# BjarkeHautop/bayesSSM

Hardware: AMD Instinct MI355X
Metric: particle-steps/sec (N x T), bootstrap filter (higher is better)
Workload: dtype f64; 1 GPU; BASELINE C2: linear-Gaussian SSM, bootstrap filter, T=1000, N=1048576, SISR + systematic resampling, return_particles=FALSE, device generator; per_gpu=one independent filter replica per GPU (no data-path collective), backend=single process

## Files before the change

bayesssm_amd/_lib.py:

```python
import contextlib
import ctypes as C
import os
import threading

_HERE = os.path.dirname(os.path.abspath(__file__))
LIB_PATH = os.environ.get("BAYESSSM_AMD_LIB") or os.path.join(_HERE, "libbayesssm_amd.so")

OK, ERR_NEGATIVE, ERR_ZERO_SUM, ERR_LENGTH, ERR_ARG, ERR_HIP, ERR_CAPACITY = range(7)
MODEL = {"lg": 0, "ar1sin": 1, "sir": 2, "lgmv": 3, "rnet": 6}
MV_OBS_MODEL = {"gaussian": 3, "poisson": 4, "logvar": 5}
RN_OBS_MODEL = {"poisson": 6, "negbin": 7}
ALGORITHM = {"BPF": 0, "APF": 1, "RMPF": 2}
RESAMPLE_ALGORITHM = {"SIS": 0, "SISR": 1, "SISAR": 2}
RESAMPLE_FN = {"stratified": 0, "systematic": 1, "multinomial": 2, "multinomial_r": 3}
TRANSFORM = {"identity": 0, "log": 1, "logit": 2}
PRIOR = {"normal": 0, "exponential": 1, "uniform": 2, "flat": 3, "halfnormal": 4}


class BssmError(RuntimeError):
    def __init__(self, status, message):
        super().__init__(message)
        self.status = status


# ... 65 lines not shown
    lib.bssm_last_error.restype = C.c_char_p
    lib.bssm_status_string.restype = C.c_char_p
    lib.bssm_status_string.argtypes = [C.c_int]
    lib.bssm_ctx_stream.restype = C.c_void_p
    lib.bssm_ctx_stream.argtypes = [C.c_void_p]
    lib.bssm_ctx_create.argtypes = [C.c_int, C.c_longlong, C.c_int, C.POINTER(C.c_void_p)]
    lib.bssm_ctx_destroy.argtypes = [C.c_void_p]
    lib.bssm_ctx_destroy.restype = None
    lib.bssm_ctx_synchronize.argtypes = [C.c_void_p]
    lib.bssm_ctx_set_profile.argtypes = [C.c_void_p, C.c_int]
    lib.bssm_ctx_set_option.argtypes = [C.c_void_p, C.c_int, C.c_int]
    lib.bssm_ctx_get_stamps.argtypes = [C.c_void_p, C.c_void_p]
    if hasattr(lib, "bssm_ctx_fused_stats"):
        lib.bssm_ctx_fused_stats.argtypes = [C.c_void_p, C.c_void_p]
        lib.bssm_ctx_fused_stamps.argtypes = [C.c_void_p, C.c_void_p]
    if hasattr(lib, "bssm_ctx_multi_stats"):
        lib.bssm_ctx_multi_stats.argtypes = [C.c_void_p, C.c_void_p]
    lib.bssm_ctx_get_profile.argtypes = [C.c_void_p, C.c_int, C.c_void_p, C.c_void_p, C.c_void_p]
    lib.bssm_resample_ex.argtypes = [C.c_void_p, C.c_int, C.c_int, C.c_void_p, C.c_int, C.c_void_p,
                                     C.c_void_p, C.c_void_p, C.c_void_p]
    lib.bssm_resample_systematic.argtypes = [C.c_void_p, C.c_int, C.c_void_p, C.c_int, C.c_double, C.c_void_p]
    lib.bssm_resample_stratified.argtypes = [C.c_void_p, C.c_int, C.c_void_p, C.c_int, C.c_void_p, C.c_void_p]
    lib.bssm_resample_multinomial.argtypes = [C.c_void_p, C.c_int, C.c_void_p, C.c_int, C.c_void_p, C.c_void_p]
    lib.bssm_resample_multinomial_r.argtypes = [C.c_void_p, C.c_int, C.c_void_p, C.c_int, C.c_void_p, C.c_void_p]
    lib.bssm_resample_device.argtypes = [C.c_void_p, C.c_int, C.c_int, C.c_void_p, C.c_int, C.c_double,
                                         C.c_void_p, C.c_void_p, C.c_void_p]
    lib.bssm_resample_device_status.argtypes = [C.c_void_p]
    lib.bssm_pf_run.argtypes = [C.c_void_p, C.POINTER(PfConfig), C.POINTER(PfResult)]
    lib.bssm_pf_noise_shape.argtypes = [C.c_int, C.c_int, C.c_void_p, C.POINTER(C.c_int), C.POINTER(C.c_int)]
    lib.bssm_dump_normals.argtypes = [C.c_void_p, C.c_ulonglong, C.c_ulonglong, C.c_int, C.c_int, C.c_longlong, C.c_void_p]
# ... 23 lines not shown
        lib.bssm_pf_run_batch_tv.argtypes = [C.c_void_p, C.POINTER(PfConfig), C.c_int, C.c_void_p, C.c_void_p, C.c_void_p,
                                             C.POINTER(MvTvBatch), C.POINTER(PfBatchResult)]
    _lib = lib
    return lib


EXPORTED_SYMBOLS = [
    "bssm_ctx_create", "bssm_ctx_destroy", "bssm_last_error", "bssm_status_string", "bssm_device_count",
    "bssm_ctx_synchronize", "bssm_ctx_stream", "bssm_resample_systematic", "bssm_resample_stratified",
    "bssm_resample_multinomial", "bssm_resample_device", "bssm_resample_device_status", "bssm_resample_ex",
    "bssm_pf_run", "bssm_pf_noise_shape", "bssm_dump_normals", "bssm_dump_uniforms", "bssm_dump_move_draws",
    "bssm_ctx_set_profile", "bssm_ctx_get_profile", "bssm_ctx_set_option", "bssm_ctx_get_stamps", "bssm_pmmh_chain",
    "bssm_resample_multinomial_r",
    "bssm_pf_run_batch", "bssm_pf_run_batch_tv", "bssm_pf_batch_max_particles", "bssm_pf_batch_max_particles_mv", "bssm_pf_batch_max_particles_rn", "bssm_rn_nb_tables", "bssm_pmmh_chains_batch", "bssm_pmmh_chain_draws",
    "bssm_pf_run_sharded", "bssm_pf_weigh_resample", "bssm_ctx_fused_stats", "bssm_ctx_fused_stamps", "bssm_dump_normals_mv", "bssm_dump_move_draws_mv", "bssm_pf_run_multi", "bssm_pmmh_chains_multi",
    "bssm_ctx_multi_stats", "bssm_dump_rpois", "bssm_dump_rbinom", "bssm_dump_rgamma",
]


def check(status):
    if status != OK:
        lib = load()
        msg = lib.bssm_last_error().decode() or lib.bssm_status_string(status).decode()
        raise BssmError(status, msg)


class Context:

    def __init__(self, device=0, max_particles=1 << 20, max_dim=1):
        lib = load()
        if lib.bssm_device_count() <= 0:
# ... 8 lines not shown
        if os.environ.get("BAYESSSM_AMD_FUSED") is not None:
            check(lib.bssm_ctx_set_option(h, 9, int(os.environ["BAYESSSM_AMD_FUSED"])))
        if os.environ.get("BAYESSSM_AMD_FUSED_PREFETCH") is not None:
            check(lib.bssm_ctx_set_option(h, 10, int(os.environ["BAYESSSM_AMD_FUSED_PREFETCH"])))

    @property
    def handle(self):
        return self._h

    def synchronize(self):
        check(load().bssm_ctx_synchronize(self._h))

    OPTIONS = {"record_window": 1, "batch_literal_max": 2, "stage_expansion": 3, "inkernel_resolve": 4, "debug_stop": 5, "fuse_step": 6, "renormalize": 7, "recompute_lw": 8, "fused": 9, "fused_prefetch": 10,
               "force_fallback": 11, "fused_tag": 12, "mv_y_missing": 13, "rn_leaps": 14, "fused_early_max": 0}

    QUALIFIERS = {"rn_method": OPTIONS["rn_leaps"] + 1, "rn_noise": OPTIONS["rn_leaps"] + 2}

    def set_option(self, name, value):
        check(load().bssm_ctx_set_option(self._h, self.OPTIONS[name] if name in self.OPTIONS else self.QUALIFIERS[name], int(value)))
        self._set_options[name] = int(value)

    @contextlib.contextmanager
    def mv_y_missing(self, skip):
        if not skip:
            yield
            return
        before = self._set_options.get("mv_y_missing", 0)
        self.set_option("mv_y_missing", 1)
        try:
            yield
        finally:
# ... 21 lines not shown
                    self.set_option("rn_method", method)
                if noise != before_noise:
                    self.set_option("rn_noise", noise)
                yield
            finally:
                if self._set_options.get("rn_noise", 0) != before_noise:
                    self.set_option("rn_noise", before_noise)
                if self._set_options.get("rn_method", 0) != before:
                    self.set_option("rn_method", before)

    def fused_stats(self):
        out = (C.c_longlong * 4)()
        check(load().bssm_ctx_fused_stats(self._h, out))
        return {"runs": out[0], "launches": out[1], "stand_downs": out[2], "timeouts": out[3]}

    def multi_stats(self):
        out = (C.c_longlong * 2)()
        check(load().bssm_ctx_multi_stats(self._h, out))
        return {"lockstep": out[0], "sequential": out[1]}

    def set_profile(self, enable):
        check(load().bssm_ctx_set_profile(self._h, 1 if enable else 0))

    def get_profile(self):
        n = 64
        names = (C.c_char_p * n)()
        ms = (C.c_double * n)()
        cnt = (C.c_longlong * n)()
        k = load().bssm_ctx_get_profile(self._h, n, names, ms, cnt)
        return {names[i].decode(): {"ms": ms[i], "launches": cnt[i]} for i in range(k)}
# ... 43 lines not shown
```

bayesssm_amd/csrc/bssm_api.hip:

```cpp
#include <hip/hip_runtime.h>
#include <hip/hip_ext.h>
#include <math.h>
#include <stdio.h>
#include <string.h>
#include <string>
#include <vector>
#include <map>
#include <algorithm>
#include "kernels.hip.h"
#include "fused.hip.h"
#include "mv.hip.h"
#include "rnet.hip.h"
#include "multi.hip.h"
#include <atomic>
#include "../../include/bayesssm_amd.h"

using namespace bssm;

static thread_local std::string g_err;

#define HIPCHK(expr)                                                                      \
    do {                                                                                  \
        hipError_t e__ = (expr);                                                          \
        if (e__ != hipSuccess) {                                                          \
// ... 17 lines not shown
    BlockRec *brec = nullptr, *brec_p = nullptr;
    SideList *side = nullptr, *side_p = nullptr;
    uint64_t* cin = nullptr;
    DevState* st = nullptr;
    unsigned long long* gmax_cur = nullptr;
    int sh_boff = 0, sh_nloc = 0;
    int opt_window = 0;
    int opt_batch_lit_max = 384;
    int opt_stage = 1;
    int opt_inkernel_resolve = 1;
    int opt_renormalize = 1;
    int opt_recompute_lw = 1;
    int opt_fuse_step = 0;
    int opt_debug_stop = 0;
    int opt_fused_prefetch = 0;
    int opt_fused_early_max = 1;
    int opt_force_fallback = 0;
    int opt_mv_y_missing = 0;
    int opt_rn_leaps = 0;
    int opt_rn_noise = 0;
    int opt_rn_method = 0;
    int opt_fused = 1;
    FusedWs* fz = nullptr; uint32_t fz_tag = 0; bool fz_ok = false;
    long long fz_launches = 0, fz_runs = 0, fz_bails = 0, fz_timeouts = 0;
    long long multi_lockstep = 0, multi_sequential = 0;
    std::map<std::string, std::pair<void*, size_t>> pool;
    hipEvent_t ev0 = nullptr, ev1 = nullptr;
    void* h_stage = nullptr; size_t h_stage_bytes = 0;
    bool profile = false;
    std::map<std::string, ProfEntry> prof;
// ... 169 lines not shown
    switch (option) {
        case BSSM_OPT_RN_NOISE: c->opt_rn_noise = value; break;
        case BSSM_OPT_RN_LEAPS: c->opt_rn_leaps = value; break;
        case BSSM_OPT_RN_METHOD: c->opt_rn_method = value; break;
        case BSSM_OPT_RECORD_WINDOW: c->opt_window = value; break;
        case BSSM_OPT_BATCH_LITERAL_MAX: c->opt_batch_lit_max = value; break;
        case BSSM_OPT_STAGE_EXPANSION: c->opt_stage = value; break;
        case BSSM_OPT_INKERNEL_RESOLVE: c->opt_inkernel_resolve = value; break;
        case BSSM_OPT_DEBUG_STOP: c->opt_debug_stop = value; break;
        case BSSM_OPT_FUSE_STEP: c->opt_fuse_step = value; break;
        case BSSM_OPT_RECOMPUTE_LW: c->opt_recompute_lw = value ? 1 : 0; break;
        case BSSM_OPT_RENORMALIZE: c->opt_renormalize = value ? 1 : 0; break;
        case BSSM_OPT_FUSED: c->opt_fused = value < 0 ? 0 : (value > 2 ? 2 : value); break;
        case BSSM_OPT_FUSED_PREFETCH: c->opt_fused_prefetch = value ? 1 : 0; break;
        case BSSM_OPT_FUSED_EARLY_MAX: c->opt_fused_early_max = value ? 1 : 0; break;
        case BSSM_OPT_MV_Y_MISSING: c->opt_mv_y_missing = value ? 1 : 0; break;
        case BSSM_OPT_FORCE_FALLBACK: {
            if (value < 0 || value > (FF_SERIAL_WALK | FF_GENERAL_LINK | FF_SUM_PASS_ONLY)) ARGFAIL("bssm_ctx_set_option: force_fallback takes the bits 1 | 2 | 4");
            const int32_t v = value;
            HIPCHK(hipSetDevice(c->device));
            HIPCHK(hipMemcpyAsync(&c->st->force_fallback, &v, sizeof(v), hipMemcpyHostToDevice, c->stream));
            HIPCHK(hipStreamSynchronize(c->stream));
            c->opt_force_fallback = value;
            break;
        }
        case BSSM_OPT_FUSED_TAG: {
            if (!c->fz) ARGFAIL("bssm_ctx_set_option: this context has no fused workspace");
            HIPCHK(hipSetDevice(c->device));
            HIPCHK(hipMemsetAsync(c->fz, 0, sizeof(FusedWs), c->stream));
            HIPCHK(hipStreamSynchronize(c->stream));
// ... 542 lines not shown
            if (cfg->return_particles)
                LAUNCH(c, "k_record_history", k_record_history, (unsigned)((N + 255) / 256), 256, 0, X0, c->w, N, dim,
                       (double*)d_ph + (size_t)i * N * dim, (double*)d_wh + (size_t)i * N, c->st);
        };
        if (fused) {
            for (int step = 1; step < gap; step++) { launch_step_model(c, cfg->model, true, 0, false, X0, N, B, par, yi, noise(ktrans)); ktrans++; }
            FusedArgs g;
            g.xin = X0; g.N = N; g.nblk = B; g.par = par; g.y = yi; g.trans = (gap >= 1) ? 1 : 0; g.ns = noise(gap >= 1 ? ktrans : 0);
            if (gap >= 1) ktrans++;
            g.obs_i = i; g.resample_algorithm = resample_algorithm; g.threshold = threshold;
            g.ess_out = (double*)d_ess; g.llh_out = (double*)d_llh; g.resampled_out = (int*)d_resampled;
            g.w_out = cfg->return_particles ? c->w : nullptr;
            g.lim = c->opt_window > 0 ? c->opt_window : rec_window(N);
            g.force_fallback = c->opt_force_fallback;
            g.early_max = c->opt_fused_early_max;
            ApplyArgs& a = g.a;
            a.w = c->w; a.nw = N; a.ain_p = c->ain_p; a.cin = c->cin; a.lim = g.lim; a.n = (int)N;
            a.u_base = (const double*)d_ur; a.u_stride = u_stride; a.key = key;
            a.anc_out = (int*)d_anc; a.anc_stride = N; a.cum_out = nullptr;
            a.xsrc = X0; a.xdst = X1; a.dim = 1; a.xstride = N; a.auxsrc = nullptr; a.auxdst = nullptr;
            a.se_part = se_row;
            a.nstage = (c->opt_stage && !d_anc) ? 1 : 0; a.lead = 0; a.last = B - 1;
            a.step_model = -1; a.step_par = par; a.step_y = 0; a.step_ns = g.ns; a.step_lw = nullptr;
            g.ws = c->fz; g.tag = ++c->fz_tag;
            if (g.tag == 0) {
                HIPCHK(hipMemsetAsync(c->fz, 0, sizeof(FusedWs), c->stream));
                g.tag = c->fz_tag = 1;
            }
            g.znext = nullptr; g.znext_call = 0;
            if (z_ready) { g.ns.arr = z_ready; z_ready = nullptr; }
// ... 611 lines not shown
    HIPCHK(hipMemcpy(out, c->fz->pubt, sizeof(c->fz->pubt), hipMemcpyDeviceToHost));
    return BSSM_OK;
}

extern "C" int bssm_ctx_fused_waket(bssm_ctx* c, long long* out )
{
    if (!c || !out || !c->fz) ARGFAIL("bssm_ctx_fused_waket: NULL argument");
    HIPCHK(hipMemcpy(out, c->fz->waket, sizeof(c->fz->waket), hipMemcpyDeviceToHost));
    return BSSM_OK;
}

extern "C" int bssm_ctx_fused_stats(bssm_ctx* c, long long* out )
{
    if (!c || !out) ARGFAIL("bssm_ctx_fused_stats: NULL argument");
    out[0] = c->fz_runs; out[1] = c->fz_launches; out[2] = c->fz_bails; out[3] = c->fz_timeouts;
    return BSSM_OK;
}

extern "C" int bssm_ctx_multi_stats(bssm_ctx* c, long long* out )
{
    if (!c || !out) ARGFAIL("bssm_ctx_multi_stats: NULL argument");
    out[0] = c->multi_lockstep; out[1] = c->multi_sequential;
    return BSSM_OK;
}

extern "C" int bssm_pf_run_multi(bssm_ctx* const* ctxs, int n_filters, const bssm_pf_config* cfg, const double* thetas,
                                 const unsigned long long* seeds, const unsigned long long* streams, bssm_pf_batch_result* res)
{
    if (!ctxs || !cfg || !res || !thetas || !seeds || !streams) ARGFAIL("bssm_pf_run_multi: NULL argument");
    const int F = n_filters;
// ... 1003 lines not shown
```

bayesssm_amd/csrc/fused.hip.h:

```cpp
#pragma once
#include "kernels.hip.h"

namespace bssm {

typedef unsigned long long fz_u64;
#define BSSM_RLX_AGENT __ATOMIC_RELAXED, __HIP_MEMORY_SCOPE_AGENT

constexpr int FZ_MAXB = 2 * NT;
constexpr int FZ_MINB = 256;
constexpr int FZ_KREC = 8;
constexpr int FZ_KSIDE = (int)(sizeof(SideEntry) / 4);
constexpr int FZ_NREP = 16;
constexpr int FZ_MAXSIDE = 16;
constexpr uint32_t FLAG_FUSED_BAIL = 8u, FLAG_FUSED_TIMEOUT = 16u;
constexpr uint32_t FZ_ST_DOIT = 1u, FZ_ST_DEAD = 2u, FZ_ST_STOP = 4u, FZ_ST_BAIL = 8u;
constexpr long long FZ_TIMEOUT_TICKS = 2000000ll;

struct FusedWs {
    fz_u64 e1[6][FZ_MAXB];
    fz_u64 c1[FZ_NREP][16];
    fz_u64 m1[FZ_NREP][16];
    fz_u64 s1[FZ_NREP][16];
    fz_u64 a1[2][FZ_MAXB];
    fz_u64 e2[FZ_KREC][FZ_MAXB];
    fz_u64 c2[FZ_NREP][16];
    fz_u64 e3[FZ_KREC][FZ_MAXB];
    fz_u64 c3[FZ_NREP][16];
    fz_u64 a3[2][FZ_MAXB];
    fz_u64 side_w[FZ_MAXB][FZ_MAXSIDE][FZ_KSIDE];
    fz_u64 side_p[FZ_MAXB][FZ_MAXSIDE][FZ_KSIDE];
    BlockRec brec_priv[2][MAXB];
    SideList side_priv[2][FZ_MAXB];
    long long stamps[2][24];
    long long startt[FZ_MAXB];
    long long endt[FZ_MAXB];
    long long waket[5][FZ_MAXB];
    long long pubt[4][FZ_MAXB];
};

#ifdef BSSM_DEV_STAMPS
#define FZ_STAMP(k) do { if (fz_stamper) g.ws->stamps[fz_row][k] = clock64(); } while (0)
#else
#define FZ_STAMP(k) do { } while (0)
#endif

__device__ __forceinline__ fz_u64 fz_gran(uint32_t tag, uint32_t v) { return ((fz_u64)tag << 32) | v; }
__device__ __forceinline__ void fz_put(fz_u64* g, uint32_t tag, uint32_t v) { __hip_atomic_store(g, fz_gran(tag, v), BSSM_RLX_AGENT); }
__device__ __forceinline__ void fz_put64(fz_u64* g, uint32_t tag, uint64_t v) { fz_put(g, tag, (uint32_t)v); fz_put(g + 1, tag, (uint32_t)(v >> 32)); }
__device__ __forceinline__ void fz_put64x(fz_u64* g, int stride, uint32_t tag, uint64_t v) { fz_put(g, tag, (uint32_t)v); fz_put(g + stride, tag, (uint32_t)(v >> 32)); }
__device__ __forceinline__ fz_u64 fz_get(const fz_u64* g) { return __hip_atomic_load(g, BSSM_RLX_AGENT); }

__device__ __forceinline__ void fz_encode(const BlockRec& br, uint32_t (&w)[FZ_KREC])
// ... 67 lines not shown
            for (int k = 0; k < EL; k++) c = c + terms[tt * EL + k];
        }
        atomicAdd((unsigned long long*)&st->stat_serial_walks, 1ull);
        atomicAdd((unsigned long long*)&st->stat_literal_terms, (unsigned long long)EB);
    }
    __syncthreads();
}
__device__ __forceinline__ LaneTerms fz_lane_terms(const double (&v)[EL])
{
    LaneTerms r;
#pragma unroll
    for (int k = 0; k < EL; k++) r.a[k] = v[k];
    return r;
}

struct FusedRecSink {
    fz_u64* rec_planes;
    fz_u64* side_base;
    int bidx; uint32_t tag;
    double* terms; DevState* st;
    __device__ __forceinline__ void rec(const BlockRec& br) const
    {
        uint32_t w[FZ_KREC];
        fz_encode(br, w);
#pragma unroll
        for (int k = 0; k < FZ_KREC; k++) fz_put(rec_planes + (size_t)k * FZ_MAXB + bidx, tag, w[k]);
    }
    __device__ __forceinline__ void side(int k, const SideEntry& e) const
    {
        if (k >= FZ_MAXSIDE) return;
        uint32_t w[FZ_KSIDE];
// ... 2 lines not shown
#pragma unroll
        for (int q = 0; q < FZ_KSIDE; q++) fz_put(dst + q, tag, w[q]);
    }
    __device__ __forceinline__ void literal(uint64_t* tin, uint64_t cin, const double (&v)[EL]) const { fz_block_literal(tin, cin, terms, fz_lane_terms(v), st); }
};

struct FusedArgs {
    const double* xin;
    long long N; int nblk;
    ModelPar par; double y; NoiseSrc ns; int trans;
    int obs_i, resample_algorithm; double threshold;
    double* ess_out; double* llh_out; int* resampled_out;
    double* w_out;
    int lim;
    int force_fallback;
    int early_max;
    ApplyArgs a;
    FusedWs* ws; uint32_t tag;
    double* znext; uint32_t znext_call;
};

struct FusedSmem {
    double red[16]; double redq[16];
    uint32_t slot[16];
    int bail;
    int book; double ess1;
};

template <int NG>
__device__ __forceinline__ bool fz_gather(const fz_u64* planes, int c0, int c1, uint32_t tag, const FzClock& clk, int* bail, uint32_t (&w0)[NG], uint32_t (&w1)[NG])
// ... 452 lines not shown
        double acc0 = 0.0;
#pragma unroll
        for (int r = 0; r < EL; r++) {
            const long long j = b0 + t + NT * r;
            if (j < N) { const double x0 = xa[t + NT * r]; g.a.xdst[j] = x0; acc0 += x0 * wa[t + NT * r]; }
        }
        acc0 = block_sum(acc0, sm.sh4);
        if (t == 0) g.a.se_part[bidx] = acc0;
        book_late();
        fz_draw_next(g, j0, N);
        return;
    }
    if (status & FZ_ST_STOP) { book_late(); return; }
    FZ_STAMP(6);
    FusedRecSink sink; sink.bidx = bidx; sink.tag = g.tag; sink.terms = lx; sink.st = st;
    {
        BlockScan bsw;
        block_scan<MODE_W>(sm, v, a_in, g.lim, bsw);
        __syncthreads();
        sink.rec_planes = &g.ws->e2[0][0]; sink.side_base = &g.ws->side_w[0][0][0];
        block_record_tail<MODE_W, 11>(sm, tin, bsw, v, a_in, g.lim, st, 0, false, sink);
    }
    FZ_STAMP(7); FZ_PUBT(1);
    book_late();
    if (!resolver) fz_draw_next(g, j0, N);
    ResolveSmem& rs = *reinterpret_cast<ResolveSmem*>(dyn);
    uint64_t* cin_lds = reinterpret_cast<uint64_t*>(reinterpret_cast<char*>(dyn) + ((sizeof(ResolveSmem) + 15) / 16) * 16);
    if (resolver) {
        __syncthreads();
        bool bail = false;
        const uint64_t fin = fz_resolve_duty<MODE_W, false>(sm, rs, fs, g, st, clk, nullptr, bail);
        uint32_t stw = 0;
        if (bail) { stw = FZ_ST_BAIL; if (t == 0) atomicOr(&st->flags, fs.bail == 1 ? FLAG_FUSED_TIMEOUT : FLAG_FUSED_BAIL); }
        else {
// ... 24 lines not shown
        if (fs.slot[2] & (FZ_ST_BAIL | FZ_ST_STOP)) return;
        total = b2d(mk64(fs.slot[0], fs.slot[1]));
    }
    FZ_STAMP(11); FZ_WAKE(1);
    const double a_in_p = a_in / total;
#pragma unroll
    for (int k = 0; k < EL; k++) v[k] = v[k] / total;
    BlockScan bs;
#ifdef BSSM_DEV_STAMPS
    const bool xstamper = (t == 0 && bidx == B / 4);
    const int xdbg = 99;
    if (xstamper) st->stamps[2][10] = clock64();
#else
    const bool xstamper = false; const int xdbg = 0;
#endif
    block_scan<MODE_P>(sm, v, a_in_p, g.lim, bs);
    __syncthreads();
#ifdef BSSM_DEV_STAMPS
    if (xstamper) st->stamps[2][11] = clock64();
#endif
    sink.rec_planes = &g.ws->e3[0][0]; sink.side_base = &g.ws->side_p[0][0][0];
    block_record_tail<MODE_P, 3>(sm, tin, bs, v, a_in_p, g.lim, st, xdbg, xstamper, sink);
#ifdef BSSM_DEV_STAMPS
    if (xstamper) { st->stamps[2][9] = clock64(); st->stamps[2][8] = bs.nb; }
#endif
    FZ_STAMP(12); FZ_PUBT(2);
    uint64_t cinb = 0;
    if (resolver) {
        __syncthreads();
        bool bail = false;
        (void)fz_resolve_duty<MODE_P, true>(sm, rs, fs, g, st, clk, cin_lds, bail);
        uint32_t stp = 0;
        if (bail) { stp = FZ_ST_BAIL; if (t == 0) atomicOr(&st->flags, fs.bail == 1 ? FLAG_FUSED_TIMEOUT : FLAG_FUSED_BAIL); }
        for (int b = t; b < B; b += NT) fz_put64x(&g.ws->a3[0][b], FZ_MAXB, g.tag, bail ? 0ull : cin_lds[b]);
// ... 56 lines not shown
```

bayesssm_amd/csrc/kernels.hip.h:

```cpp
#pragma once
#include <hip/hip_runtime.h>
#include <stdint.h>
#include <math.h>
#include "seqsum.h"
#include "rng.h"

namespace bssm {

#ifndef BSSM_NT
#define BSSM_NT 256
#endif
#ifndef BSSM_EL
#define BSSM_EL 8
#endif
constexpr int NT = BSSM_NT;
constexpr int EL = BSSM_EL;
constexpr int NWV = NT / 64;
static_assert(NT * EL == 2048 && (NT == 256 || NT == 512) , "a scan workgroup covers 2048 terms with 4 or 8 waves");
constexpr int EB = NT * EL;
constexpr int MAXB = 2048;

typedef double v2d_nt __attribute__((ext_vector_type(2)));
#ifndef BSSM_ST_W
#define BSSM_ST_W 0
// ... 579 lines not shown
    int j = 0;
#pragma unroll 1
    for (; j < nent; j++) {
        const bool bad = (sv + w.nref) >= w.range;
        const uint32_t lo = (uint32_t)sv;
        const uint64_t k01 = (lo & 1u) ? w.K1 : w.K0, k23 = (lo & 1u) ? w.K3 : w.K2;
        const uint64_t out = ((sv & ~3ull) >> (w.sh & 63)) + ((lo & 2u) ? k23 : k01);
        if (__builtin_amdgcn_readlane((int)bad, j)) break;
        if (lane == j) { my_s = sv; my_out = out; }
        sv = readlane_u64(out, j);
    }
    s = sv;
    return j;
}

__device__ __forceinline__ int64_t shfl_up_i64(int64_t v, int off)
{
    int lo = (int)(uint32_t)(uint64_t)v, hi = (int)(uint32_t)((uint64_t)v >> 32);
    lo = __shfl_up(lo, off, 64); hi = __shfl_up(hi, off, 64);
    return (int64_t)(((uint64_t)(uint32_t)hi << 32) | (uint32_t)lo);
}

struct SegSmem {
    Pure wagg[16]; int wflag[16]; int wnb[16]; Pure wcarry[17]; int wsegbase[17];
    Pure bnd_excl[MAXBND]; Rec bnd_rec[MAXBND]; int bnd_lane[MAXBND]; uint64_t bnd_ent[MAXBND];
    double bnd_terms[MAXBND][EL];
    uint64_t seg_start[MAXBND + 1];
    int red_min[NWV][2], red_max[NWV][2];
    uint64_t segbase[MAXBND + 1];
    int wlastb[16];
// ... 146 lines not shown
{
    double c = b2d(in);
    for (long long j = j0; j < j1; j++) c = c + term_at<MODE>(w, nw, total, j);
    return d2b(c);
}

struct BlockScan {
    Rec leaf;
    Pure pleaf;
    Pure exc;
    Pure last_seg;
    bool isb;
    int seg, nb;
};

template <int MODE>
__device__ __forceinline__ void block_scan(SegSmem& sm, const double (&v)[EL], double a_in, int lim, BlockScan& bs)
{
    double ts = 0.0;
#pragma unroll
    for (int k = 0; k < EL; k++) ts += v[k];
    const double h = a_in + block_excl_scan(ts, sm.sh4);
    bs.leaf = chunk_record_fixed<EL>(v, h, lim);
    bs.isb = bs.leaf.kind != REC_PURE;
    bs.pleaf.d0 = (int64_t)(bs.leaf.o[0] - bs.leaf.base);
    bs.pleaf.d1 = (int64_t)(bs.leaf.o[1] - (bs.leaf.base + 1));
    bool prev_b = false;
    bs.exc = seg_excl_scan<NT / 64>(sm, bs.pleaf, bs.isb, bs.seg, bs.nb, bs.last_seg, &prev_b);
    if (!bs.isb && prev_b && bs.seg <= MAXBND) sm.segbase[bs.seg] = bs.leaf.base;
    if (bs.isb && bs.seg < MAXBND) {
        Rec& d = sm.bnd_rec[bs.seg];
        d.base = bs.leaf.base; d.o[0] = bs.leaf.o[0]; d.o[1] = bs.leaf.o[1]; d.o[2] = bs.leaf.o[2]; d.o[3] = bs.leaf.o[3];
        d.kind = bs.leaf.kind; d.lo = bs.leaf.lo; d.hi = bs.leaf.hi; d.pad = 0;
        sm.bnd_excl[bs.seg].d0 = bs.exc.d0; sm.bnd_excl[bs.seg].d1 = bs.exc.d1; sm.bnd_lane[bs.seg] = threadIdx.x;
#pragma unroll
        for (int q = 0; q < EL; q++) sm.bnd_terms[bs.seg][q] = v[q];
    }
}

template <int MODE>
__device__ __forceinline__ bool block_resolve(SegSmem& sm, const BlockScan& bs, uint64_t cin, int lim,
                                              const double* __restrict__ w, long long nw, double total, long long b0,
                                              uint64_t& ent)
{
    const int t = threadIdx.x;
    if (t == 0) sm.fail = (bs.nb > MAXBND) ? 1 : 0;
    __syncthreads();
    if (t < 64 && bs.nb == 0) {
        if (t == 0) sm.seg_start[0] = cin;
    } else if (t < 64 && bs.nb <= MAXBND) {
        const int lane = t, nb = bs.nb;
        Rec rec = rec_identity(0);
        Pure ex; ex.d0 = 0; ex.d1 = 0;
        if (lane < nb) { rec = sm.bnd_rec[lane]; ex = sm.bnd_excl[lane]; }
        const StepFn fn = stepfn_build(ex, rec);
        uint64_t s = cin, my_s = 0, my_out = 0;
        const WalkFn wfn = walkfn_from(fn, lane < nb);
        const int j0 = walk_chain_regs(wfn, nb, s, my_s, my_out);
        for (int j = j0; j < nb; j++) {
            bool ok;
            uint64_t o = stepfn_apply(fn, s, ok);
            if (!__builtin_amdgcn_readlane((int)ok, j)) {
                double c = b2d(pure_step(ex, s));
#pragma unroll
                for (int q = 0; q < EL; q++) c = c + sm.bnd_terms[j][q];
                o = d2b(c);
            }
            if (lane == j) { my_s = s; my_out = o; }
            const int olo = __builtin_amdgcn_readlane((int)(uint32_t)o, j), ohi = __builtin_amdgcn_readlane((int)(uint32_t)(o >> 32), j);
            s = ((uint64_t)(uint32_t)ohi << 32) | (uint32_t)olo;
        }
        const uint64_t my_ent = pure_step(ex, my_s);
        if (lane == 0) sm.seg_start[0] = cin;
        if (lane < nb) { sm.bnd_ent[lane] = my_ent; sm.seg_start[lane + 1] = my_out; }
    }
    __syncthreads();
    if (bs.nb > MAXBND) return false;
    bool ok = true;
    if (bs.isb) ent = sm.bnd_ent[bs.seg];
    else {
        ent = pure_step(bs.exc, sm.seg_start[bs.seg]);
        const int64_t diff = (int64_t)(ent - bs.leaf.base);
        ok = (diff >= -(int64_t)lim) && (diff <= (int64_t)lim);
    }
    if (!ok) sm.fail = 1;
    __syncthreads();
    return sm.fail == 0;
}

template <int MODE>
__device__ __attribute__((noinline)) void block_literal(uint64_t* tin , uint64_t cin, const double* __restrict__ w,
                                              long long nw, double total, long long b0, DevState* st)
{
    if (threadIdx.x == 0) {
// ... 77 lines not shown
}

__device__ __forceinline__ Rec pure_to_rec(const Pure& p, uint64_t base, long long lo, long long hi)
{
    Rec r; r.pad = 0; r.base = base & ~3ull; r.kind = REC_PURE;
    r.o[0] = r.base + (uint64_t)p.d0; r.o[1] = r.base + 1 + (uint64_t)p.d1;
    r.o[2] = r.base + 2 + (uint64_t)p.d0; r.o[3] = r.base + 3 + (uint64_t)p.d1;
    const long long L = -(1ll << 30), H = (1ll << 30);
    r.lo = (int32_t)(lo < L ? L : (lo > H ? H : lo));
    r.hi = (int32_t)(hi < L ? L : (hi > H ? H : hi));
    return r;
}

template <int MODE>
struct GlobalRecSink {
    BlockRec* brec; SideList* sides; int bidx, bstride;
    const double* w; long long nw; double total; long long b0; DevState* st;
    __device__ __forceinline__ void rec(const BlockRec& br) const { store_brec(brec, bidx, br, bstride); }
    __device__ __forceinline__ void side(int k, const SideEntry& e) const { this->side_list()[k] = e; }
    __device__ __forceinline__ SideEntry* side_list() const { return sides[bidx].e; }
    __device__ __forceinline__ void literal(uint64_t* tin, uint64_t cin, const double (&)[EL]) const { block_literal<MODE>(tin, cin, w, nw, total, b0, st); }
};

template <int MODE, int STAMPCOL, class Sink>
__device__ __forceinline__ void block_record_tail(SegSmem& sm, uint64_t* tin, const BlockScan& bs, const double (&v)[EL], const double a_in,
                                                  const int lim, DevState* st, const int dbg, const bool stamper, const Sink& sink)
{
    const int t = threadIdx.x;
    (void)dbg; (void)stamper;
    BSSM_STAMP(st, dbg, 2, 12, stamper);
    const uint64_t hb0 = d2b(a_in) & ~3ull;
    if (a_in == 0.0) {
        uint64_t ent;
        bool good = block_resolve<MODE>(sm, bs, 0ull, lim, nullptr, 0, 1.0, 0, ent);
        if (!good) { sink.literal(tin, 0ull, v); ent = tin[t]; }
        if (t == NT - 1) {
            double c = b2d(ent);
#pragma unroll
            for (int k = 0; k < EL; k++) c = c + v[k];
            BlockRec br; br.prefix = rec_abs(d2b(c)); br.tail_from = NT; br.nside = 0;
            sink.rec(br);
        }
        return;
    }
    int fb = NT;
    uint64_t seg1_base = 0;
    if (bs.nb > 0) { fb = sm.bnd_lane[0]; seg1_base = sm.segbase[1]; }
    int mn[2] = {WSAT, WSAT}, mx[2] = {-WSAT, -WSAT};
    if (!bs.isb && bs.seg <= 1) {
// ... 1855 lines not shown
```

bayesssm_amd/csrc/seqsum.h:

```cpp
#pragma once
#include <stdint.h>
#include <string.h>

#if defined(__HIPCC__)
#define BSSM_HD __host__ __device__ __forceinline__
#else
#define BSSM_HD inline
#endif

namespace bssm {

BSSM_HD uint64_t d2b(double x) { uint64_t b; memcpy(&b, &x, 8); return b; }
BSSM_HD double b2d(uint64_t b) { double x; memcpy(&x, &b, 8); return x; }

enum : int32_t { REC_PURE = 0, REC_X1 = 1, REC_ABS = 2, REC_HARD = 3 };

struct Rec {
    uint64_t base;
    uint64_t o[4];
    int32_t kind;
    int32_t lo, hi;
    int32_t pad;
};

// ... 158 lines not shown
    bool ok = true;
    for (int s = 0; s < 4; s++) r.o[s] = rec_step(g, f.o[s], ok);
    if (!ok) return rec_hard(f.base);
    r.kind = (f.kind == REC_X1 || g.kind == REC_X1) ? REC_X1 : REC_PURE;
    r.lo = (int32_t)lo; r.hi = (int32_t)hi;
    return r;
}

BSSM_HD uint64_t run_literal(const double* v, int L, int vs, uint64_t in)
{
    double c = b2d(in);
    for (int k = 0; k < L; k++) c = c + v[k * vs];
    return d2b(c);
}


#if defined(__HIPCC__)
__host__ __device__ __attribute__((noinline))
#endif
inline int32_t count_le_systematic_exact(double c, int32_t n, double U, double g)
{
    const double dn = (double)n;
    int64_t t = (g < 0) ? 0 : (g >= dn ? (int64_t)n : (int64_t)g + 1);
    if (t > n) t = n;
    while (t < n && !((((double)t + U) / dn) > c)) t++;
    while (t > 0 && ((((double)(t - 1) + U) / dn) > c)) t--;
    return (int32_t)t;
}

BSSM_HD int32_t count_le_systematic(double c, int32_t n, double U)
// ... 50 lines not shown
```

include/bayesssm_amd.h:

```cpp
#ifndef BAYESSSM_AMD_H
#define BAYESSSM_AMD_H

#ifdef __cplusplus
extern "C" {
#endif

#define BSSM_OK 0
#define BSSM_ERR_NEGATIVE_WEIGHT 1
#define BSSM_ERR_ZERO_SUM 2
#define BSSM_ERR_LENGTH 3
#define BSSM_ERR_ARG 4
#define BSSM_ERR_HIP 5
#define BSSM_ERR_CAPACITY 6

#define BSSM_MODEL_LG 0
#define BSSM_MODEL_AR1SIN 1
#define BSSM_MODEL_SIR 2
#define BSSM_MODEL_LGMV 3
#define BSSM_MODEL_LGMV_POIS 4
#define BSSM_MODEL_LGMV_LOGVAR 5
#define BSSM_MODEL_RNET 6
#define BSSM_MODEL_RNET_NB 7

#define BSSM_BPF 0
// ... 34 lines not shown
#define BSSM_OPT_STAGE_EXPANSION 3
#define BSSM_OPT_INKERNEL_RESOLVE 4
#define BSSM_OPT_DEBUG_STOP 5
#define BSSM_OPT_RENORMALIZE 7
#define BSSM_OPT_RECOMPUTE_LW 8
#define BSSM_OPT_FUSED 9
#define BSSM_OPT_FUSED_PREFETCH 10
#define BSSM_OPT_FORCE_FALLBACK 11
#define BSSM_OPT_FUSED_TAG 12
#define BSSM_OPT_FUSED_EARLY_MAX 0
#define BSSM_OPT_FUSE_STEP 6
#define BSSM_OPT_MV_Y_MISSING 13
#define BSSM_OPT_RN_LEAPS 14
#define BSSM_OPT_RN_METHOD (BSSM_OPT_RN_LEAPS + 1)
#define BSSM_OPT_RN_NOISE (BSSM_OPT_RN_LEAPS + 2)
int bssm_ctx_set_option(bssm_ctx* ctx, int option, int value);
int bssm_ctx_get_stamps(bssm_ctx* ctx, long long* out );
int bssm_ctx_fused_stats(bssm_ctx* ctx, long long* out );
int bssm_ctx_multi_stats(bssm_ctx* ctx, long long* out );
int bssm_ctx_fused_stamps(bssm_ctx* ctx, long long* out );

int bssm_resample_systematic(bssm_ctx* ctx, int n, const double* weights, int nw, double U, int* indices_out);
int bssm_resample_stratified(bssm_ctx* ctx, int n, const double* weights, int nw, const double* U, int* indices_out);
int bssm_resample_multinomial(bssm_ctx* ctx, int n, const double* weights, int nw, const double* U, int* indices_out);
int bssm_resample_multinomial_r(bssm_ctx* ctx, int n, const double* weights, int nw, const double* U, int* indices_out);

int bssm_resample_device(bssm_ctx* ctx, int kind, int n, const double* d_weights, int nw,
                         double U_scalar, const double* d_U, int* d_indices_out, double* d_cum_out);
int bssm_resample_device_status(bssm_ctx* ctx);

int bssm_resample_ex(bssm_ctx* ctx, int kind, int n, const double* weights, int nw, const double* U,
                     int* indices_out, double* cum_out, long long* stats);

// ... 155 lines not shown
```

Before: 23.10 billion particle-steps/s.

## Precompute literal head prefix states in spare wave during fused block scan

In the fused resample kernel, block 0 stages the first K lanes' weight terms and a lane in the last wave sequentially computes exact literal prefix states during the block scan. The boundary-chain walk in block_resolve then starts after those head boundaries, and head lanes take their entry states directly from the precomputed array. The aim is to shorten the serial chain walk on the critical path of block 0 by overlapping part of it with the scan. This adds a serial per-pass computation on one lane, an atomic counter, extra shared staging, and new handover logic that has to be correct. It is on by default.

```diff
diff --git a/bayesssm_amd/_lib.py b/bayesssm_amd/_lib.py
--- a/bayesssm_amd/_lib.py
+++ b/bayesssm_amd/_lib.py
@@ -103,6 +103,8 @@
     if hasattr(lib, "bssm_ctx_fused_stats"):
         lib.bssm_ctx_fused_stats.argtypes = [C.c_void_p, C.c_void_p]
         lib.bssm_ctx_fused_stamps.argtypes = [C.c_void_p, C.c_void_p]
+    if hasattr(lib, "bssm_ctx_fused_head_literal"):
+        lib.bssm_ctx_fused_head_literal.argtypes = [C.c_void_p, C.c_void_p]
     if hasattr(lib, "bssm_ctx_multi_stats"):
         lib.bssm_ctx_multi_stats.argtypes = [C.c_void_p, C.c_void_p]
     lib.bssm_ctx_get_profile.argtypes = [C.c_void_p, C.c_int, C.c_void_p, C.c_void_p, C.c_void_p]
@@ -156,7 +158,7 @@
     "bssm_resample_multinomial_r",
     "bssm_pf_run_batch", "bssm_pf_run_batch_tv", "bssm_pf_batch_max_particles", "bssm_pf_batch_max_particles_mv", "bssm_pf_batch_max_particles_rn", "bssm_rn_nb_tables", "bssm_pmmh_chains_batch", "bssm_pmmh_chain_draws",
     "bssm_pf_run_sharded", "bssm_pf_weigh_resample", "bssm_ctx_fused_stats", "bssm_ctx_fused_stamps", "bssm_dump_normals_mv", "bssm_dump_move_draws_mv", "bssm_pf_run_multi", "bssm_pmmh_chains_multi",
-    "bssm_ctx_multi_stats", "bssm_dump_rpois", "bssm_dump_rbinom", "bssm_dump_rgamma",
+    "bssm_ctx_multi_stats", "bssm_dump_rpois", "bssm_dump_rbinom", "bssm_dump_rgamma", "bssm_ctx_fused_head_literal",
 ]
 
 
@@ -195,7 +197,7 @@
     OPTIONS = {"record_window": 1, "batch_literal_max": 2, "stage_expansion": 3, "inkernel_resolve": 4, "debug_stop": 5, "fuse_step": 6, "renormalize": 7, "recompute_lw": 8, "fused": 9, "fused_prefetch": 10,
                "force_fallback": 11, "fused_tag": 12, "mv_y_missing": 13, "rn_leaps": 14, "fused_early_max": 0}
 
-    QUALIFIERS = {"rn_method": OPTIONS["rn_leaps"] + 1, "rn_noise": OPTIONS["rn_leaps"] + 2}
+    QUALIFIERS = {"rn_method": OPTIONS["rn_leaps"] + 1, "rn_noise": OPTIONS["rn_leaps"] + 2, "fused_head_literal": OPTIONS["rn_leaps"] + 3}
 
     def set_option(self, name, value):
         check(load().bssm_ctx_set_option(self._h, self.OPTIONS[name] if name in self.OPTIONS else self.QUALIFIERS[name], int(value)))
@@ -247,6 +249,11 @@
         check(load().bssm_ctx_fused_stats(self._h, out))
         return {"runs": out[0], "launches": out[1], "stand_downs": out[2], "timeouts": out[3]}
 
+    def fused_head_literal_passes(self):
+        out = (C.c_longlong * 1)()
+        check(load().bssm_ctx_fused_head_literal(self._h, out))
+        return out[0]
+
     def multi_stats(self):
         out = (C.c_longlong * 2)()
         check(load().bssm_ctx_multi_stats(self._h, out))
diff --git a/bayesssm_amd/csrc/bssm_api.hip b/bayesssm_amd/csrc/bssm_api.hip
--- a/bayesssm_amd/csrc/bssm_api.hip
+++ b/bayesssm_amd/csrc/bssm_api.hip
@@ -55,6 +55,7 @@
     int opt_fuse_step = 0;
     int opt_debug_stop = 0;
     int opt_fused_prefetch = 0;
+    int opt_fused_head_literal = 1;
     int opt_fused_early_max = 1;
     int opt_force_fallback = 0;
     int opt_mv_y_missing = 0;
@@ -254,6 +255,7 @@
         case BSSM_OPT_FUSED: c->opt_fused = value < 0 ? 0 : (value > 2 ? 2 : value); break;
         case BSSM_OPT_FUSED_PREFETCH: c->opt_fused_prefetch = value ? 1 : 0; break;
         case BSSM_OPT_FUSED_EARLY_MAX: c->opt_fused_early_max = value ? 1 : 0; break;
+        case BSSM_OPT_FUSED_HEAD_LITERAL: c->opt_fused_head_literal = value ? 1 : 0; break;
         case BSSM_OPT_MV_Y_MISSING: c->opt_mv_y_missing = value ? 1 : 0; break;
         case BSSM_OPT_FORCE_FALLBACK: {
             if (value < 0 || value > (FF_SERIAL_WALK | FF_GENERAL_LINK | FF_SUM_PASS_ONLY)) ARGFAIL("bssm_ctx_set_option: force_fallback takes the bits 1 | 2 | 4");
@@ -826,6 +828,7 @@
             g.lim = c->opt_window > 0 ? c->opt_window : rec_window(N);
             g.force_fallback = c->opt_force_fallback;
             g.early_max = c->opt_fused_early_max;
+            g.head_literal = c->opt_fused_head_literal;
             ApplyArgs& a = g.a;
             a.w = c->w; a.nw = N; a.ain_p = c->ain_p; a.cin = c->cin; a.lim = g.lim; a.n = (int)N;
             a.u_base = (const double*)d_ur; a.u_stride = u_stride; a.key = key;
@@ -1467,6 +1470,19 @@
 {
     if (!c || !out) ARGFAIL("bssm_ctx_fused_stats: NULL argument");
     out[0] = c->fz_runs; out[1] = c->fz_launches; out[2] = c->fz_bails; out[3] = c->fz_timeouts;
+    return BSSM_OK;
+}
+
+extern "C" int bssm_ctx_fused_head_literal(bssm_ctx* c, long long* out )
+{
+    if (!c || !out) ARGFAIL("bssm_ctx_fused_head_literal: NULL argument");
+    out[0] = 0;
+    if (!c->fz) return BSSM_OK;
+    HIPCHK(hipSetDevice(c->device));
+    HIPCHK(hipStreamSynchronize(c->stream));
+    unsigned long long v = 0;
+    HIPCHK(hipMemcpy(&v, &c->fz->head_lit, sizeof(v), hipMemcpyDeviceToHost));
+    out[0] = (long long)v;
     return BSSM_OK;
 }
 
diff --git a/bayesssm_amd/csrc/fused.hip.h b/bayesssm_amd/csrc/fused.hip.h
--- a/bayesssm_amd/csrc/fused.hip.h
+++ b/bayesssm_amd/csrc/fused.hip.h
@@ -15,6 +15,12 @@
 constexpr uint32_t FLAG_FUSED_BAIL = 8u, FLAG_FUSED_TIMEOUT = 16u;
 constexpr uint32_t FZ_ST_DOIT = 1u, FZ_ST_DEAD = 2u, FZ_ST_STOP = 4u, FZ_ST_BAIL = 8u;
 constexpr long long FZ_TIMEOUT_TICKS = 2000000ll;
+#ifndef BSSM_HEAD_K
+#define BSSM_HEAD_K 9
+#endif
+constexpr int FZ_HEAD_K = BSSM_HEAD_K;
+constexpr int FZ_HEAD_LANE = NT - 64;
+static_assert(FZ_HEAD_K >= 1 && FZ_HEAD_K < NT - 64, "the literal prefix ends in front of the wave that adds it");
 
 struct FusedWs {
     fz_u64 e1[6][FZ_MAXB];
@@ -36,6 +42,7 @@
     long long endt[FZ_MAXB];
     long long waket[5][FZ_MAXB];
     long long pubt[4][FZ_MAXB];
+    fz_u64 head_lit;
 };
 
 #ifdef BSSM_DEV_STAMPS
@@ -133,7 +140,28 @@
     return r;
 }
 
+struct FzHeadMid {
+    const double* terms; uint64_t* states; FusedWs* ws; bool on; int pass;
+    __device__ __forceinline__ void operator()() const
+    {
+        if (on && threadIdx.x == FZ_HEAD_LANE) {
+#ifdef BSSM_DEV_STAMPS
+            ws->pubt[3][24 + 3 * pass] = clock64();
+#endif
+            head_literal_states<EL>(terms, FZ_HEAD_K, states);
+            atomicAdd((unsigned long long*)&ws->head_lit, 1ull);
+#ifdef BSSM_DEV_STAMPS
+            ws->pubt[3][25 + 3 * pass] = clock64();
+#endif
+        }
+    }
+};
+
 struct FusedRecSink {
+    static constexpr bool head_literal = true;
+    const uint64_t* hl;
+    __device__ __forceinline__ const uint64_t* head_states() const { return hl; }
+    __device__ __forceinline__ int head_lanes() const { return FZ_HEAD_K; }
     fz_u64* rec_planes;
     fz_u64* side_base;
     int bidx; uint32_t tag;
@@ -166,6 +194,7 @@
     double* w_out;
     int lim;
     int force_fallback;
+    int head_literal;
     int early_max;
     ApplyArgs a;
     FusedWs* ws; uint32_t tag;
@@ -648,10 +677,23 @@
     if (status & FZ_ST_STOP) { book_late(); return; }
     FZ_STAMP(6);
     FusedRecSink sink; sink.bidx = bidx; sink.tag = g.tag; sink.terms = lx; sink.st = st;
+    const bool hlit = g.head_literal && bidx == 0;
+    double* hterms = lx + EB;
+    uint64_t* hstates = reinterpret_cast<uint64_t*>(hterms + FZ_HEAD_K * EL);
+    static_assert(EB + FZ_HEAD_K * EL + FZ_HEAD_K + 1 <= EB + CAPX, "the literal prefix fits the staging area");
+    FzHeadMid hmid; hmid.terms = hterms; hmid.states = hstates; hmid.ws = g.ws; hmid.on = hlit; hmid.pass = 0;
+    sink.hl = hlit ? hstates : nullptr;
     {
         BlockScan bsw;
-        block_scan<MODE_W>(sm, v, a_in, g.lim, bsw);
-        __syncthreads();
+        if (hlit && t < FZ_HEAD_K) {
+#pragma unroll
+            for (int k = 0; k < EL; k++) hterms[t * EL + k] = v[k];
+        }
+        block_scan<MODE_W>(sm, v, a_in, g.lim, bsw, hmid);
+        __syncthreads();
+#ifdef BSSM_DEV_STAMPS
+        if (hlit && t == 0) g.ws->pubt[3][26] = clock64();
+#endif
         sink.rec_planes = &g.ws->e2[0][0]; sink.side_base = &g.ws->side_w[0][0][0];
         block_record_tail<MODE_W, 11>(sm, tin, bsw, v, a_in, g.lim, st, 0, false, sink);
     }
@@ -706,10 +748,16 @@
 #else
     const bool xstamper = false; const int xdbg = 0;
 #endif
-    block_scan<MODE_P>(sm, v, a_in_p, g.lim, bs);
+    if (hlit && t < FZ_HEAD_K) {
+#pragma unroll
+        for (int k = 0; k < EL; k++) hterms[t * EL + k] = v[k];
+    }
+    hmid.pass = 1;
+    block_scan<MODE_P>(sm, v, a_in_p, g.lim, bs, hmid);
     __syncthreads();
 #ifdef BSSM_DEV_STAMPS
     if (xstamper) st->stamps[2][11] = clock64();
+    if (hlit && t == 0) g.ws->pubt[3][29] = clock64();
 #endif
     sink.rec_planes = &g.ws->e3[0][0]; sink.side_base = &g.ws->side_p[0][0][0];
     block_record_tail<MODE_P, 3>(sm, tin, bs, v, a_in_p, g.lim, st, xdbg, xstamper, sink);
diff --git a/bayesssm_amd/csrc/kernels.hip.h b/bayesssm_amd/csrc/kernels.hip.h
--- a/bayesssm_amd/csrc/kernels.hip.h
+++ b/bayesssm_amd/csrc/kernels.hip.h
@@ -617,6 +617,25 @@
     return j;
 }
 
+__device__ __forceinline__ int walk_chain_regs_from(const WalkFn& w, int nent, uint64_t& s, uint64_t& my_s, uint64_t& my_out, const int jb)
+{
+    const int lane = threadIdx.x & 63;
+    uint64_t sv = readlane_u64(s, 0);
+    int j = jb;
+#pragma unroll 1
+    for (; j < nent; j++) {
+        const bool bad = (sv + w.nref) >= w.range;
+        const uint32_t lo = (uint32_t)sv;
+        const uint64_t k01 = (lo & 1u) ? w.K1 : w.K0, k23 = (lo & 1u) ? w.K3 : w.K2;
+        const uint64_t out = ((sv & ~3ull) >> (w.sh & 63)) + ((lo & 2u) ? k23 : k01);
+        if (__builtin_amdgcn_readlane((int)bad, j)) break;
+        if (lane == j) { my_s = sv; my_out = out; }
+        sv = readlane_u64(out, j);
+    }
+    s = sv;
+    return j;
+}
+
 __device__ __forceinline__ int64_t shfl_up_i64(int64_t v, int off)
 {
     int lo = (int)(uint32_t)(uint64_t)v, hi = (int)(uint32_t)((uint64_t)v >> 32);
@@ -793,13 +812,15 @@
     int seg, nb;
 };
 
-template <int MODE>
-__device__ __forceinline__ void block_scan(SegSmem& sm, const double (&v)[EL], double a_in, int lim, BlockScan& bs)
+struct NoMid { __device__ __forceinline__ void operator()() const {} };
+template <int MODE, class Mid = NoMid>
+__device__ __forceinline__ void block_scan(SegSmem& sm, const double (&v)[EL], double a_in, int lim, BlockScan& bs, const Mid mid = Mid())
 {
     double ts = 0.0;
 #pragma unroll
     for (int k = 0; k < EL; k++) ts += v[k];
     const double h = a_in + block_excl_scan(ts, sm.sh4);
+    mid();
     bs.leaf = chunk_record_fixed<EL>(v, h, lim);
     bs.isb = bs.leaf.kind != REC_PURE;
     bs.pleaf.d0 = (int64_t)(bs.leaf.o[0] - bs.leaf.base);
@@ -817,10 +838,10 @@
     }
 }
 
-template <int MODE>
+template <int MODE, bool HEAD = false>
 __device__ __forceinline__ bool block_resolve(SegSmem& sm, const BlockScan& bs, uint64_t cin, int lim,
                                               const double* __restrict__ w, long long nw, double total, long long b0,
-                                              uint64_t& ent)
+                                              uint64_t& ent, const uint64_t* hl = nullptr, const int hk = 0)
 {
     const int t = threadIdx.x;
     if (t == 0) sm.fail = (bs.nb > MAXBND) ? 1 : 0;
@@ -832,10 +853,23 @@
         Rec rec = rec_identity(0);
         Pure ex; ex.d0 = 0; ex.d1 = 0;
         if (lane < nb) { rec = sm.bnd_rec[lane]; ex = sm.bnd_excl[lane]; }
+        int js = 0;
+        uint64_t s = cin;
+        if constexpr (HEAD) {
+            if (hl) {
+                const int bl = (lane < nb) ? sm.bnd_lane[lane] : NT;
+                js = __popcll(__ballot(bl < hk));
+                const uint64_t behind = hl[bl < hk ? bl + 1 : 0];
+                if (js) s = readlane_u64(behind, js - 1);
+            }
+        }
+        const uint64_t s_in = s;
         const StepFn fn = stepfn_build(ex, rec);
-        uint64_t s = cin, my_s = 0, my_out = 0;
+        uint64_t my_s = 0, my_out = 0;
         const WalkFn wfn = walkfn_from(fn, lane < nb);
-        const int j0 = walk_chain_regs(wfn, nb, s, my_s, my_out);
+        int j0;
+        if constexpr (HEAD) j0 = walk_chain_regs_from(wfn, nb, s, my_s, my_out, js);
+        else j0 = walk_chain_regs(wfn, nb, s, my_s, my_out);
         for (int j = j0; j < nb; j++) {
             bool ok;
             uint64_t o = stepfn_apply(fn, s, ok);
@@ -850,13 +884,16 @@
             s = ((uint64_t)(uint32_t)ohi << 32) | (uint32_t)olo;
         }
         const uint64_t my_ent = pure_step(ex, my_s);
-        if (lane == 0) sm.seg_start[0] = cin;
-        if (lane < nb) { sm.bnd_ent[lane] = my_ent; sm.seg_start[lane + 1] = my_out; }
+        if (lane == 0) sm.seg_start[js] = s_in;
+        if (lane >= js && lane < nb) { sm.bnd_ent[lane] = my_ent; sm.seg_start[lane + 1] = my_out; }
     }
     __syncthreads();
     if (bs.nb > MAXBND) return false;
     bool ok = true;
-    if (bs.isb) ent = sm.bnd_ent[bs.seg];
+    bool inhead = false;
+    if constexpr (HEAD) inhead = hl && t < hk;
+    if (inhead) ent = hl[t];
+    else if (bs.isb) ent = sm.bnd_ent[bs.seg];
     else {
         ent = pure_step(bs.exc, sm.seg_start[bs.seg]);
         const int64_t diff = (int64_t)(ent - bs.leaf.base);
@@ -964,6 +1001,7 @@
 
 template <int MODE>
 struct GlobalRecSink {
+    static constexpr bool head_literal = false;
     BlockRec* brec; SideList* sides; int bidx, bstride;
     const double* w; long long nw; double total; long long b0; DevState* st;
     __device__ __forceinline__ void rec(const BlockRec& br) const { store_brec(brec, bidx, br, bstride); }
@@ -982,7 +1020,9 @@
     const uint64_t hb0 = d2b(a_in) & ~3ull;
     if (a_in == 0.0) {
         uint64_t ent;
-        bool good = block_resolve<MODE>(sm, bs, 0ull, lim, nullptr, 0, 1.0, 0, ent);
+        bool good;
+        if constexpr (Sink::head_literal) good = block_resolve<MODE, true>(sm, bs, 0ull, lim, nullptr, 0, 1.0, 0, ent, sink.head_states(), sink.head_lanes());
+        else good = block_resolve<MODE>(sm, bs, 0ull, lim, nullptr, 0, 1.0, 0, ent);
         if (!good) { sink.literal(tin, 0ull, v); ent = tin[t]; }
         if (t == NT - 1) {
             double c = b2d(ent);
diff --git a/bayesssm_amd/csrc/seqsum.h b/bayesssm_amd/csrc/seqsum.h
--- a/bayesssm_amd/csrc/seqsum.h
+++ b/bayesssm_amd/csrc/seqsum.h
@@ -196,6 +196,33 @@
     return d2b(c);
 }
 
+template <int L>
+BSSM_HD void head_literal_states(const double* terms , int K, uint64_t* st )
+{
+    double c = 0.0, a[L], b[L];
+#pragma unroll
+    for (int k = 0; k < L; k++) a[k] = terms[k];
+    for (int i = 0; i < K; i++) {
+        const int nx = (i + 1 < K) ? i + 1 : i;
+    #pragma unroll
+    for (int k = 0; k < L; k++) b[k] = terms[nx * L + k];
+        st[i] = d2b(c);
+    #pragma unroll
+    for (int k = 0; k < L; k++) c = c + a[k];
+    #pragma unroll
+    for (int k = 0; k < L; k++) a[k] = b[k];
+    }
+    st[K] = d2b(c);
+}
+
+BSSM_HD int head_handover(const int* bnd_lane, int nb, int K, const uint64_t* st, uint64_t& s)
+{
+    int js = 0;
+    while (js < nb && bnd_lane[js] < K) js++;
+    s = js ? st[bnd_lane[js - 1] + 1] : st[0];
+    return js;
+}
+
 
 #if defined(__HIPCC__)
 __host__ __device__ __attribute__((noinline))
diff --git a/include/bayesssm_amd.h b/include/bayesssm_amd.h
--- a/include/bayesssm_amd.h
+++ b/include/bayesssm_amd.h
@@ -72,9 +72,11 @@
 #define BSSM_OPT_RN_LEAPS 14
 #define BSSM_OPT_RN_METHOD (BSSM_OPT_RN_LEAPS + 1)
 #define BSSM_OPT_RN_NOISE (BSSM_OPT_RN_LEAPS + 2)
+#define BSSM_OPT_FUSED_HEAD_LITERAL (BSSM_OPT_RN_LEAPS + 3)
 int bssm_ctx_set_option(bssm_ctx* ctx, int option, int value);
 int bssm_ctx_get_stamps(bssm_ctx* ctx, long long* out );
 int bssm_ctx_fused_stats(bssm_ctx* ctx, long long* out );
+int bssm_ctx_fused_head_literal(bssm_ctx* ctx, long long* out );
 int bssm_ctx_multi_stats(bssm_ctx* ctx, long long* out );
 int bssm_ctx_fused_stamps(bssm_ctx* ctx, long long* out );
 
```

Result: no change. 23.27 billion particle-steps/s (median of 6 runs) (+0.8%).
